# AppleHolic/pytorch_sound

Measured on AMD Instinct MI355X. Metric: audio-sec/s STFT+mel+fwd/bwd, higher is better.
Workload: dtype bf16; 1 GPU; configs[1]: Conv1d separator (4 x ResBlock1, C=256, on 513-bin magnitude), 22.05 kHz, STFT 1024/256, 80 mel, batch 32 x 2 s per GPU, Adam, bf16 autocast; global_batch=32, parallelism=dp1, model_params=5520386

## Files before the change

include/psnd.h:

```cpp
#ifndef PSND_H
#define PSND_H

#include <stdint.h>
#include <stddef.h>

#ifdef __cplusplus
extern "C" {
#endif

#define PSND_OK 0
#define PSND_E_ARG (-1)
#define PSND_E_SHAPE (-2)
#define PSND_E_HIP (-3)
#define PSND_E_UNSUPPORTED (-4)

#define PSND_FRAMING_CENTER 0
#define PSND_FRAMING_HIFIGAN 1
#define PSND_FRAMING_NONE 2

int psnd_version(void);
const char *psnd_last_error(void);
#ifdef PSND_LAB
void psnd_env_refresh(void);
#endif
// ... 89 lines not shown
typedef struct psnd_chain_pair {
    const void *W1;
    const float *bias1;
    float act1_slope;
    void *mid_out;
    const void *W2;
    const float *bias2;
    int off1, dstep1, off2, dstep2;
    float act2_slope;
    void *out_raw, *out_act;
    const void *M1, *M2;
    float m1_slope, m2_slope;
} psnd_chain_pair;
int psnd_conv1d_cl_chain_rows(int C, int k, int n_pairs, const int *taps);
int psnd_conv1d_cl_chain_plan(int C, int k, int n_pairs, const int *taps, int64_t R, int *mr_out);
int psnd_conv1d_cl_chain(const void *A, const void *res, const psnd_chain_pair *pairs, int n_pairs, int64_t N, int Lp, int L, int HP,
                         int C, int k, void *stream);
void psnd_conv_chain_stats(long long *out2);
int psnd_to_cl_nfk(const float *x_nfk, int64_t N, int K, int64_t F, int Lp, int HP, int Cp, int preop, void *out, void *stream);
int64_t psnd_mask_head_l1_blocks_nfk(int64_t N, int64_t F, int K);
int psnd_mask_head_l1_fwd_nfk(const void *y, const float *mag_nfk, const float *ref_nfk, int64_t N, int K, int64_t F, int Lp, int HP, int Cp,
                              float *est_nfk, double *part, void *stream);
int psnd_mask_head_l1_bwd_nfk(const float *gest_nfk, const float *mag_nfk, const void *y, const float *est_nfk, const float *ref_nfk,
                              const float *g, float coef, int64_t N, int K, int64_t F, int Lp, int HP, int Cp, void *gy, void *stream);
int psnd_mel_fwd_nfk(const float *mag_nfk, int64_t N, int64_t F, int M, int K, const void *mel_plan, int log_kind, float log_offset,
                     float pre_clamp_min, float clamp_lo, float clamp_hi, float *out, float *mel_lin, void *stream);
int psnd_mel_bwd_nfk(const float *gout, const float *mel_lin, int64_t N, int64_t F, int M, int K, const void *mel_plan, int log_kind,
                     float log_offset, float pre_clamp_min, float clamp_lo, float clamp_hi, float *gmag_nfk, void *stream);
int psnd_mel_l1_fwd_nfk(const float *mag_nfk, int64_t N, int64_t F, int M, int K, const void *mel_plan, int log_kind, float log_offset,
                        float pre_clamp_min, float clamp_lo, float clamp_hi, const float *ref, float *mel_lin, double *part, void *stream);
int psnd_mel_l1_bwd_nfk(const float *ref, const float *mel_lin, const float *g, float coef, int64_t N, int64_t F, int M, int K,
                        const void *mel_plan, int log_kind, float log_offset, float pre_clamp_min, float clamp_lo, float clamp_hi,
                        float *gmag_nfk, void *stream);
int64_t psnd_mask_head_l1_blocks(int64_t N, int64_t T, int Cp);
int psnd_mask_head_l1_fwd(const void *y, const float *mag, const float *ref, int64_t N, int C, int64_t T, int Lp, int HP, int Cp,
                          float *est, double *part, void *stream);
int psnd_mask_head_l1_bwd(const float *gest, const float *mag, const void *y, const float *est, const float *ref, const float *g,
                          float coef, int64_t N, int C, int64_t T, int Lp, int HP, int Cp, void *gy, void *stream);
int64_t psnd_mel_l1_blocks(int64_t N, int64_t F, int M);
int psnd_mel_l1_fwd(const float *mag, int64_t N, int64_t F, int M, int K, const void *mel_plan, int log_kind, float log_offset,
                    float pre_clamp_min, float clamp_lo, float clamp_hi, const float *ref, float *mel_lin, double *part, void *stream);
int psnd_mel_l1_bwd(const float *ref, const float *mel_lin, const float *g, float coef, int64_t N, int64_t F, int M, int K,
                    const void *mel_plan, int log_kind, float log_offset, float pre_clamp_min, float clamp_lo, float clamp_hi,
                    float *gmag, void *stream);
int psnd_nan_flag(const float *x, int64_t n, float *flag, void *stream);
int psnd_l1_loss_combine(const double *const *parts, const int64_t *nb, const double *scale, int terms, float *out, float *nan_flag, void *stream);
int psnd_conv_stats(int64_t *out4, int reset);
int psnd_conv_pair_stats(int64_t *out4, int reset);
int psnd_conv1d_cl_wgrad(const void *G1, const void *G2, const void *GM, float g2_slope, const void *xa, int64_t N,
                         int Lp, int Ca, int Cb, int k, int off0, int dstep, float *gw_part, float *gbias_part,
                         void *g_out, void *stream);
int psnd_conv1d_prep(const float *v, const float *g, const float *bias, int Cout, int Cin, int k, int Cb, int Ca,
                     void *wf, void *wb, float *bias_padded, void *stream);
int psnd_convtr1d_prep(const float *v, const float *g, const float *bias, int Cin, int Cout, int K, int stride, int Cr, int Cip,
                       void *wf, void *wb, float *bias_rep, void *stream);
int psnd_convtr1d_prep_multi(const void *descs_dev, int n, int total_blocks, void *stream);
int psnd_convtr1d_cl_fwd(const void *xa, const void *wf, const float *bias_rep, int64_t N, int Lp, int L, int HP, int Cip, int Cr,
                         int stride, int padding, int LpO, int HPO, float act_slope, void *out_raw, void *out_act, void *stream);
int psnd_convtr1d_cl_wgrad_splits(int64_t N, int Lp, int Cip, int Cr, int stride);
int psnd_convtr1d_cl_bwd(const void *g_raw, const void *g_act, const void *act, float act_slope, const void *wb, const void *xa,
                         int64_t N, int Lp, int L, int HP, int Cip, int Cr, int stride, int padding, int LpO, int HPO, void *gx,
                         void *g_eff, float *gw_part, void *stream);
int psnd_convtr1d_wnorm_bwd(const float *gw_part, int splits, const float *v, const float *g, int Cin, int Cout, int K, int stride,
                            int Cr, int Cip, float *gv, float *gg, void *stream);
int psnd_cl_mean_act_fwd(const void *a, const void *b, const void *c, const void *d, int count, float slope, void *out, int64_t n,
                         void *stream);
// ... 223 lines not shown
```

pytorch_sound_amd/cl.py:

```python
import ctypes
from collections import namedtuple
from pytorch_sound_amd import _switches as _sw
import weakref

import torch

from . import _lib
from ._lib import lib, ptr, on

ALIGN_C = 32


def round_up(x, m):
    return (x + m - 1) // m * m


class CLShape:

    def __init__(self, N, L, HP):
        self.N, self.L, self.HP = int(N), int(L), int(HP)
        self.Lp = round_up(self.L + 2 * self.HP, 8)

    @property
    def R(self):
# ... 344 lines not shown
        s = _PARAM_STREAM[dev.index] = torch.cuda.Stream(device=dev)
    return s



def branch_streams(dev, n):
    pool = _BRANCH_STREAMS.setdefault(dev.index, [])
    while len(pool) < n:
        pool.append(torch.cuda.Stream(device=dev))
    return pool[:n]


_WGRAD_STREAMS = {}


def _wgrad_streams(dev):
    if _sw.lab('PSND_CL_BWD_SPLIT', '0') != '1' or not _pair_enabled() or not AUTO_SECTIONS:
        return []
    n = int(_sw.lab('PSND_CL_WGRAD_STREAMS', '3'))
    pool = _WGRAD_STREAMS.setdefault(dev.index, [])
    while len(pool) < n:
        pool.append(torch.cuda.Stream(device=dev))
    return pool[:n]


def _pair_enabled():
    return _sw.lab('PSND_CL_PAIR', '1') != '0'


_Step = namedtuple('_Step', 'Cout Cin k Ca Cb dil pad slope has_res has_bias role')
_Conv = namedtuple('_Conv', 'inp wf bp res Ca Cb k off0 dil oslope raw act')
_Pair = namedtuple('_Pair', 'inp1 wf1 bp1 slope1 mid wf2 bp2 res C k off1 dstep1 off2 dstep2 oslope raw act')
_Chain = namedtuple('_Chain', 'inp1 res C k pairs')
_B = namedtuple('_B', 'G1 G2 am slope wb inp Ca Cb k pad dil gx g_out ep_mask ep_slope ep_res gw gbp S')
_W = namedtuple('_W', 'G1 G2 am slope inp Ca Cb k off0 dil gw gbp S')
_Side = namedtuple('_Side', 'w')
_PairB = namedtuple('_PairB', 'G wb2 m1 m1s g_h wb1 m2 m2s res C k off1 dstep1 off2 dstep2 gx flush_after')
_ChainB = namedtuple('_ChainB', 'pairs')
_PB = namedtuple('_PB', 'G wb2 m1 m1s g_h wb1 m2 m2s C k pad2 dil2 pad1 dil1 gx gw gbp lag')
_PBFlush = namedtuple('_PBFlush', 'lag')
_Lag = namedtuple('_Lag', 'g xa off0 dstep gw gbp C k')
_WBatch = namedtuple('_WBatch', 'conv G inp off0 dstep')


def _chain_takes(pairs):
    taps = [t for p in pairs for t in (p.off1, p.dstep1, p.off2, p.dstep2)]
    return lib().psnd_conv1d_cl_chain_rows(pairs[0].C, pairs[0].k, len(pairs), (ctypes.c_int * len(taps))(*taps)) >= 32


def _chain_pairs_bwd(plan, rows):
    mx = int(_sw.lab('PSND_CL_CHAIN_BWD', _sw.lab('PSND_CL_CHAIN', '3')))
    if mx < 2 or rows > 8192:
        return plan
    out = []
    for e in plan:
        if isinstance(e, _PairB) and e.C == 256 and e.res is e.G:
            c = out[-1] if out and isinstance(out[-1], _ChainB) else None
            if (c is not None and len(c.pairs) < mx and c.pairs[-1].gx is e.G and c.pairs[-1].k == e.k
                    and _chain_takes(c.pairs + [e])):
                c.pairs.append(e)
                continue
            out.append(_ChainB([e]))
        else:
            out.append(e)
    return [c.pairs[0] if isinstance(c, _ChainB) and len(c.pairs) == 1 else c for c in out]

# ... 269 lines not shown

class MeanActCL(torch.autograd.Function):

    @staticmethod
    def forward(ctx, slope, *rs):
        n = len(rs)
        if not 1 <= n <= 4:
            raise _lib.PsndError('MeanActCL: 1..4 branches, got %d' % n)
        rs = [r.contiguous() for r in rs]
        for r in rs:
            _need(r, torch.bfloat16)
        out = torch.empty_like(rs[0])
        ps = [ptr(r) for r in rs] + [None] * (4 - n)
        with on(out.device) as hip:
            hip.psnd_cl_mean_act_fwd(ps[0], ps[1], ps[2], ps[3], n, float(slope), out, out.numel())
        ctx.n, ctx.slope = n, float(slope)
        ctx.save_for_backward(out)
        return out

    @staticmethod
    def backward(ctx, g):
        (out,) = ctx.saved_tensors
        g = g.contiguous()
        gin = torch.empty_like(out)
        with on(out.device) as hip:
            hip.psnd_cl_mean_act_bwd(g, out, ctx.n, ctx.slope, gin, out.numel())
        return (None,) + (gin,) * ctx.n


class PrepPacks(dict):
    deferred = None

    def write_backward_packs(self):
        cache = self.deferred
        if cache is None or cache['wb_done']:
            return
        cache['wb_done'] = True
        with on(cache['dev']) as hip:
            hip.psnd_conv1d_prep_multi(cache['table'], cache['n'], cache['blocks'], cache['max_row'], 2)


def prep_all(owner, convs, defer_backward_packs=False):
    import struct
    if _sw.lab('PSND_NO_PREP_ALL') == '1':
        return None
    if any(c.weight_v.shape[1] * c.weight_v.shape[2] > 10240 for c in convs):
        return None
    key = tuple((c.weight_v.data_ptr(), c.weight_g.data_ptr(), 0 if c.bias is None else c.bias.data_ptr(),
                 tuple(c.weight_v.shape)) for c in convs)
    cache = getattr(owner, '_cl_prep_cache', None)
    if cache is None or cache['key'] != key:
        dev = convs[0].weight_v.device
        packs, recs, blk0, max_row = PrepPacks(), [], 0, 0
        for c in convs:
            Cout, Cin, k = c.weight_v.shape
            Ca, Cb = round_up(Cin, ALIGN_C), round_up(Cout, ALIGN_C)
            wf = torch.zeros((k, Cb, Ca), dtype=torch.bfloat16, device=dev)
            wb = torch.zeros((k, Ca, Cb), dtype=torch.bfloat16, device=dev)
            bp = torch.zeros(Cb, dtype=torch.float32, device=dev)
            packs[id(c)] = (wf, wb, bp)
            recs.append(struct.pack('<6Q6i', c.weight_v.data_ptr(), c.weight_g.data_ptr(),
                                    0 if c.bias is None else c.bias.data_ptr(), wf.data_ptr(), wb.data_ptr(), bp.data_ptr(),
                                    Cout, Cin, k, Cb, Ca, blk0))
            blk0 += (Cout + 7) // 8
            max_row = max(max_row, Cin * k)
        table = torch.frombuffer(bytearray(b''.join(recs)), dtype=torch.uint8).to(dev)
        cache = {'key': key, 'packs': packs, 'table': table, 'n': len(convs), 'blocks': blk0, 'max_row': max_row, 'dev': dev,
                 'wb_done': True}
        owner._cl_prep_cache = cache
    for c in convs:
        if not (c.weight_v.is_contiguous() and c.weight_g.is_contiguous() and c.weight_v.dtype == torch.float32):
            raise _lib.PsndError('prep_all: fp32 contiguous weight_v / weight_g expected')
    defer = bool(defer_backward_packs) and torch.is_grad_enabled() and _sw.lab('PSND_PREP_NO_DEFER') != '1'
    with on(cache['dev']) as hip:
        hip.psnd_conv1d_prep_multi(cache['table'], cache['n'], cache['blocks'], cache['max_row'], 1 if defer else 3)
    cache['wb_done'] = not defer
    cache['packs'].deferred = cache if defer else None
    return cache['packs']


def fused_conv(xa, conv, shape, res=None, want_raw=False, want_act=True, act_slope=0.1, prep=None):
    return FusedConvCL.apply(xa, conv.weight_v, conv.weight_g, conv.bias, res, shape, conv.dilation, want_raw, want_act,
                             act_slope, None if prep is None else prep[id(conv)])


class ResBlockCL(torch.autograd.Function):

    @staticmethod
    def forward(ctx, x, xa, shape, roles, dils, last_act_slope, want_raw, packs, *params):
        ctx.set_materialize_grads(False)
        _need(xa, torch.bfloat16)
        dev = xa.device
        n = len(dils)
        ctx.pack_owner = getattr(packs, 'owner', None)
        steps, saved, plan = [], [], []
        cur_x, cur_xa, pending = x, xa, None
        for i in range(n):
            wv, wg, b = params[3 * i:3 * i + 3]
            Cout, Cin, k = wv.shape
            role = roles[i]
            src = pending if role == 'c2' else cur_xa
            Ca, Cb = src.shape[2], round_up(Cout, ALIGN_C)
            if Ca != round_up(Cin, ALIGN_C) or (role in ('c2', 'r2') and Cb != cur_x.shape[2]):
                raise _lib.PsndError('CL conv chain: %s conv %d -> %d channels on a %d-channel buffer' % (role, Cin, Cout, Ca))
            dil = dils[i]
            pad = (k * dil - dil) // 2
            v32, g32 = wv.detach().contiguous(), wg.detach().contiguous()
            if packs is not None and packs[i] is not None:
                wf, wb, bp = packs[i]
            else:
                wf = torch.empty((k, Cb, Ca), dtype=torch.bfloat16, device=dev)
                wb = torch.empty((k, Ca, Cb), dtype=torch.bfloat16, device=dev)
                bp = torch.empty(Cb, dtype=torch.float32, device=dev)
                b32 = None if b is None else b.detach().contiguous()
                with on(dev) as hip:
                    hip.psnd_conv1d_prep(v32, g32, b32, Cout, Cin, k, Cb, Ca, wf, wb, bp)
            last = i == n - 1
            inp, slope, has_res = src, (last_act_slope if last else 0.1), role in ('c2', 'r2')
            mk = lambda: torch.empty((shape.N, shape.Lp, Cb), dtype=torch.bfloat16, device=dev)
            if role == 'c1':
                raw, act, res, oslope = None, mk(), None, slope
                pending = act
            elif role == 'tail':
                raw, act, res, oslope = mk(), None, None, 1.0
                cur_x, cur_xa = raw, None
            else:
                raw, act, res, oslope = (mk() if (not last) or want_raw else None), mk(), (cur_x if has_res else None), slope
                cur_x, cur_xa = raw, act
            c1 = plan[-1] if plan else None
            if (role == 'c2' and _pair_enabled() and isinstance(c1, _Conv) and steps[-1].role == 'c1' and c1.Ca == Ca == Cb
                    and c1.k == k and lib().psnd_conv1d_cl_pair_supported(Ca, k, c1.off0, c1.dil, -pad, dil)):
                plan[-1] = _Pair(c1.inp, c1.wf, c1.bp, c1.oslope, c1.act, wf, bp, res, Ca, k, c1.off0, c1.dil, -pad, dil, oslope, raw, act)
            else:
                plan.append(_Conv(inp, wf, bp, res, Ca, Cb, k, -pad, dil, oslope, raw, act))
            steps.append(_Step(Cout, Cin, k, Ca, Cb, dil, pad, slope, has_res, b is not None, role))
            saved += [inp, act if act is not None else inp, wb, v32, g32]
        nsec, sides = _sections(dev, shape.N, shape.N * shape.Lp)
        Nh = shape.N // nsec
        plan = _chain_pairs(plan, Nh * shape.Lp)

        def run(h):
            q = lambda t: ptr(_sec(t, h, nsec))
            with on(dev) as hip:
                for e in plan:
                    if isinstance(e, _Chain):
                        inp1, res0, C, k, pairs = e
                        arr = (_lib.ChainPair * len(pairs))()
                        for d, p in zip(arr, pairs):
                            d.W1, d.bias1, d.act1_slope, d.mid_out = p.wf1.data_ptr(), p.bp1.data_ptr(), float(p.slope1), q(p.mid)
                            d.W2, d.bias2, d.off1, d.dstep1, d.off2, d.dstep2 = p.wf2.data_ptr(), p.bp2.data_ptr(), p.off1, p.dstep1, p.off2, p.dstep2
                            d.act2_slope, d.out_raw, d.out_act = float(p.oslope), (q(p.raw) if p is pairs[-1] else None), q(p.act)
                        hip.psnd_conv1d_cl_chain(q(inp1), q(res0), ctypes.addressof(arr), len(pairs), Nh, shape.Lp, shape.L, shape.HP, C, k)
                        continue
                    if isinstance(e, _Pair):
                        inp1, wf1, bp1, slope1, mid, wf2, bp2, res, C, k, off1, dstep1, off2, dstep2, oslope, raw, act = e
                        hip.psnd_conv1d_cl_pair(q(inp1), wf1, bp1, None, 1.0, float(slope1), q(mid), wf2, bp2, None, 1.0, q(res), Nh, shape.Lp, shape.L,
                                                shape.HP, C, k, off1, dstep1, off2, dstep2, float(oslope), q(raw), q(act))
                        continue
                    inp, wf, bp, res, Ca, Cb, k, off0, dil, oslope, raw, act = e
                    hip.psnd_conv1d_cl(q(inp), None, None, 1.0, wf, bp, q(res), None, Nh, shape.Lp, shape.L, shape.HP, Ca, Cb, k, off0, dil,
                                       float(oslope), 1.0, q(raw), q(act), None)

        with torch.cuda.device(dev):
            _run_sections(dev, nsec, sides, run)
        ctx.steps, ctx.shape = steps, shape
        ctx.param_refs = params
        note_param_use(ctx, *params)
        ctx.save_for_backward(*saved)
        return cur_x, cur_xa

    @staticmethod
    def backward(ctx, g_raw, g_act):
        saved, steps, shape = ctx.saved_tensors, ctx.steps, ctx.shape
        dev = saved[0].device
        n = len(steps)
        if ctx.pack_owner is not None:
            ctx.pack_owner.write_backward_packs()
        g_raw = None if g_raw is None else g_raw.contiguous()
        g_act = None if g_act is None else g_act.contiguous()
        grads = [None] * (3 * n)
        descs, keep = [None] * n, []
        res_pending = None
        sink = GRAD_SINK if (GRAD_SINK is not None and GRAD_SINK.sink_active()) else None
        prefs = getattr(ctx, 'param_refs', None)
        early = {}

        def grad_out(i, v32, g32, Cb):
            gv = gg = gb = None
            if sink is not None and prefs is not None:
                pv, pg, pb = prefs[3 * i:3 * i + 3]
# ... 200 lines not shown
                if out:
                    sink.deliver(out)

            if sink is not None and batch:
                done_w = 0
                launches = [j for j, e in enumerate(plan) if isinstance(e, (_PairB, _ChainB))]
                L, C = len(launches), max(1, int(HANDOVER_CHUNKS))
                cut = {launches[min(L - 1, max(0, round((j + 1) * L / C) - 1))] for j in range(C - 1)} if L else set()
                ready = []
                for j, e in enumerate(plan):
                    run(0, [e])
                    ready += [ci for pe, ci in own_launch if pe is e]
                    if j not in cut:
                        continue
                    upto = (e.pairs[-1] if isinstance(e, _ChainB) else e).flush_after
                    part, done_w = wbatch[done_w:upto], upto
                    wgrad_batch(part)
                    finish(ready + [b.conv for b in part])
                    ready = []
                part = wbatch[done_w:]
                rest = [ci for ci in range(n) if descs[ci] is not None and ci not in handed and ci not in ready]
                wgrad_batch(part)
                finish(ready + rest + [b.conv for b in part])
            else:
                _run_sections(dev, nsec, sides, run)
                for sd in set(used):
                    torch.cuda.current_stream(dev).wait_stream(sd)
                wgrad_batch(wbatch)
                finish([ci for ci in range(n) if descs[ci] is not None])
        consume_param_use(ctx)
        return (g_raw, g_act, None, None, None, None, None, None) + tuple(grads)


def _block_node(convs, x, xa, shape, pairs, last_act_slope, want_raw, prep):
    params = []
    for c in convs:
        params += [c.weight_v, c.weight_g, c.bias]
    packs = None if prep is None else _PackList(prep[id(c)] for c in convs)
    if packs is not None:
        packs.owner = prep if isinstance(prep, PrepPacks) else None
    roles = pairs if isinstance(pairs, tuple) else (('c1', 'c2') * (len(convs) // 2) if pairs else ('r2',) * len(convs))
    return ResBlockCL.apply(x, xa, shape, roles, tuple(c.dilation for c in convs), last_act_slope, want_raw, packs, *params)


class _PackList(list):
    owner = None


def _use_block_node(convs, x):
    return (_sw.lab('PSND_NO_BLOCK_NODE') != '1' and x is not None and len(convs) <= 64
            and all(c.weight_v.shape[0] == c.weight_v.shape[1] for c in convs))


def conv_body_cl(head, blocks, tail, x0, shape, prep=None):
    stack = [c for b in blocks for pair in zip(b.convs1, b.convs2) for c in pair]
    if (_sw.lab('PSND_NO_BODY_NODE') == '1' or _sw.lab('PSND_NO_BLOCK_NODE') == '1' or not _stack_enabled()
            or NODE_GRANULARITY == 'block'):
        if isinstance(prep, PrepPacks):
            prep.write_backward_packs()
        x, xa = fused_conv(x0, head, shape, None, True, True, 0.1, prep)
        x, xa = resblock1_stack_cl(blocks, x, xa, shape, prep=prep)
        return fused_conv(xa, tail, shape, None, True, False, prep=prep)[0]
    convs = [head] + stack + [tail]
    roles = ('head',) + ('c1', 'c2') * (len(stack) // 2) + ('tail',)
    return _block_node(convs, None, x0, shape, roles, 0.1, True, prep)[0]


def resblock1_cl(block, x, xa, shape, last_act_slope=0.1, want_raw=True, prep=None):
    n = len(block.convs1)
    convs = [c for pair in zip(block.convs1, block.convs2) for c in pair]
    if _use_block_node(convs, x):
        return _block_node(convs, x, xa, shape, True, last_act_slope, want_raw, prep)
    for i, (c1, c2) in enumerate(zip(block.convs1, block.convs2)):
        _, ta = fused_conv(xa, c1, shape, None, False, True, 0.1, prep)
        last = i == n - 1
        x, xa = fused_conv(ta, c2, shape, x, (not last) or want_raw, True, last_act_slope if last else 0.1, prep)
    return x, xa


def resblock1_stack_cl(blocks, x, xa, shape, last_act_slope=0.1, want_raw=True, prep=None):
    convs = [c for b in blocks for pair in zip(b.convs1, b.convs2) for c in pair]
    if _use_block_node(convs, x) and _stack_enabled():
        return _block_node(convs, x, xa, shape, True, last_act_slope, want_raw, prep)
    for i, b in enumerate(blocks):
        last = i == len(blocks) - 1
        x, xa = resblock1_cl(b, x, xa, shape, last_act_slope if last else 0.1, want_raw or not last, prep)
    return x, xa


def _stack_enabled():
    return _sw.lab('PSND_NO_BLOCK_STACK') != '1' and NODE_GRANULARITY != 'block'


def resblock2_cl(block, x, xa, shape, last_act_slope=0.1, want_raw=True, prep=None):
    n = len(block.convs)
    if _use_block_node(list(block.convs), x):
        return _block_node(list(block.convs), x, xa, shape, False, last_act_slope, want_raw, prep)
    for i, c in enumerate(block.convs):
# ... 4 lines not shown
```

pytorch_sound_amd/csrc/psnd_core.hip:

```cpp
#include "psnd_common.h"

static thread_local char g_err[512] = "";

void psnd_set_error(const char *fmt, ...) {
    va_list ap;
    va_start(ap, fmt);
    vsnprintf(g_err, sizeof(g_err), fmt, ap);
    va_end(ap);
}

extern "C" int psnd_version(void) { return 151; }

extern "C" const char *psnd_last_error(void) { return g_err; }

#ifdef PSND_LAB
std::atomic<int> g_psnd_env_gen{0};
extern "C" void psnd_env_refresh(void) { g_psnd_env_gen.fetch_add(1, std::memory_order_acq_rel); }
#endif

static inline int64_t pad_of(int n_fft, int hop, int framing) {
    if (framing == PSND_FRAMING_NONE) return 0;
    return framing == PSND_FRAMING_CENTER ? n_fft / 2 : (n_fft - hop) / 2;
}

extern "C" int64_t psnd_frame_count(int64_t T, int n_fft, int hop, int framing) {
    if (T <= 0 || n_fft <= 0 || hop <= 0) return 0;
    const int64_t L = T + 2 * pad_of(n_fft, hop, framing);
    if (L < n_fft) return 0;
    return (L - n_fft) / hop + 1;
}

extern "C" int64_t psnd_frame_sample_index(int64_t f, int m, int64_t T, int n_fft, int hop, int framing) {
    int64_t i = f * hop - pad_of(n_fft, hop, framing) + m;
    if (i < 0) i = -i;
    if (i >= T) i = 2 * (T - 1) - i;
    return i;
}

extern "C" void *psnd_event_create(void) {
    hipEvent_t ev = nullptr;
    if (hipEventCreateWithFlags(&ev, hipEventDisableTiming) != hipSuccess) {
        psnd_set_error("event_create: %s", hipGetErrorString(hipGetLastError()));
        return nullptr;
    }
// ... 96 lines not shown
```

pytorch_sound_amd/csrc/psnd_nfk.hip:

```cpp
#include "psnd_common.h"

namespace {

typedef unsigned short bf16_t;
typedef __bf16 hwbf16x2 __attribute__((ext_vector_type(2)));

__device__ __forceinline__ float bf_lo(unsigned v) { return __builtin_bit_cast(float, v << 16); }
__device__ __forceinline__ float bf_hi(unsigned v) { return __builtin_bit_cast(float, v & 0xffff0000u); }
__device__ __forceinline__ unsigned pack_bf16(float lo, float hi) {
    const f32x2 v = {lo, hi};
    return __builtin_bit_cast(unsigned, __builtin_convertvector(v, hwbf16x2));
}

struct Row8 {
    float v[8];
};
__device__ __forceinline__ Row8 load8(__amdgpu_buffer_rsrc_t r, unsigned row_byte, int c0, int K, bool row_ok) {
    Row8 o;
    constexpr unsigned OOB = 0xffffffffu;
    if (c0 + 8 <= K) {
        const unsigned b = row_ok ? row_byte + 4u * (unsigned)c0 : OOB;
        const f32x4 a = __builtin_bit_cast(f32x4, __builtin_amdgcn_raw_buffer_load_b128(r, (int)b, 0, 0));
        const f32x4 c = __builtin_bit_cast(f32x4, __builtin_amdgcn_raw_buffer_load_b128(r, (int)(row_ok ? b + 16u : OOB), 0, 0));
        o.v[0] = a.x, o.v[1] = a.y, o.v[2] = a.z, o.v[3] = a.w, o.v[4] = c.x, o.v[5] = c.y, o.v[6] = c.z, o.v[7] = c.w;
    } else {
#pragma unroll
        for (int j = 0; j < 8; ++j)
            o.v[j] = __builtin_bit_cast(float, __builtin_amdgcn_raw_buffer_load_b32(r, (int)((row_ok && c0 + j < K) ? row_byte + 4u * (unsigned)(c0 + j) : OOB), 0, 0));
    }
    return o;
}
__device__ __forceinline__ void store8(__amdgpu_buffer_rsrc_t r, unsigned row_byte, int c0, int K, const float (&v)[8]) {
    if (c0 + 8 <= K) {
// ... 10 lines not shown
    const float *x;
    const float *ref;
    const float *est_in;
    const float *gest;
    const float *g;
    const bf16_t *y;
    bf16_t *out_cl;
    float *est;
    double *part;
    long long items;
    int N, F, K, Lp, HP, Cp, preop;
    unsigned tensor_bytes;
    float coef;
};

template <bool MASKBWD>
__global__ __launch_bounds__(256) void to_cl_nfk_kernel(NfkParams p) {
    const long long it = (long long)blockIdx.x * 256 + threadIdx.x;
    if (it >= p.items) return;
    const int cpr = p.Cp >> 3;
    const long long row = it / cpr;
    const int c0 = (int)(it - row * cpr) * 8;
    const int n = (int)(row / p.Lp), l = (int)(row - (long long)n * p.Lp), t = l - p.HP;
    const bool ok = t >= 0 && t < p.F;
    const unsigned rb = (unsigned)(((size_t)n * p.F + (size_t)(ok ? t : 0)) * p.K * 4);
    const int tb = (int)p.tensor_bytes;
    const __amdgpu_buffer_rsrc_t rx = make_uniform_rsrc(p.x, tb);
    float w[8];
    if constexpr (!MASKBWD) {
        const Row8 a = load8(rx, rb, c0, p.K, ok);
#pragma unroll
        for (int j = 0; j < 8; ++j) {
            float v = a.v[j];
            if (p.preop == 1) {
                const float u = 1.f + v;
                v = u == 1.f ? v : __logf(u) * __fdividef(v, u - 1.f);
            }
            w[j] = v;
        }
    } else {
        const __amdgpu_buffer_rsrc_t re = make_uniform_rsrc(p.est_in, tb), rr = make_uniform_rsrc(p.ref, tb);
        const __amdgpu_buffer_rsrc_t rg = make_uniform_rsrc(p.gest ? p.gest : p.x, p.gest ? tb : 0);
        const Row8 m = load8(rx, rb, c0, p.K, ok), e = load8(re, rb, c0, p.K, ok), r = load8(rr, rb, c0, p.K, ok), ge = load8(rg, rb, c0, p.K, ok);
        const u32x4 yq = *reinterpret_cast<const u32x4 *>(p.y + (size_t)row * p.Cp + c0);
        const float l1c = p.coef * p.g[0];
#pragma unroll
        for (int j = 0; j < 8; ++j) {
            const unsigned q = yq[j >> 1];
            const float yv = (j & 1) ? bf_hi(q) : bf_lo(q);
            const float sg = 1.f / (1.f + __expf(-yv));
            const float d = e.v[j] - r.v[j];
            const float gg = ge.v[j] + l1c * (d > 0.f ? 1.f : (d < 0.f ? -1.f : 0.f));
            w[j] = gg * m.v[j] * sg * (1.f - sg);
        }
    }
    const u32x4 o = {pack_bf16(w[0], w[1]), pack_bf16(w[2], w[3]), pack_bf16(w[4], w[5]), pack_bf16(w[6], w[7])};
    *reinterpret_cast<u32x4 *>(p.out_cl + (size_t)row * p.Cp + c0) = o;
}

__global__ __launch_bounds__(256) void mask_head_nfk_kernel(NfkParams p) {
    const long long it = (long long)blockIdx.x * 256 + threadIdx.x;
    const int cpr = (p.K + 7) >> 3;
    float acc = 0.f;
    if (it < p.items) {
        const long long row = it / cpr;
        const int c0 = (int)(it - row * cpr) * 8;
        const int n = (int)(row / p.F), t = (int)(row - (long long)n * p.F);
        const unsigned rb = (unsigned)((size_t)row * p.K * 4);
        const int tb = (int)p.tensor_bytes;
        const __amdgpu_buffer_rsrc_t rm = make_uniform_rsrc(p.x, tb), rr = make_uniform_rsrc(p.ref ? p.ref : p.x, p.ref ? tb : 0);
// ... 83 lines not shown
```

pytorch_sound_amd/models/separator.py:

```python
import torch
import torch.nn as nn
import torch.nn.functional as F

from pytorch_sound_amd.models import register_model, register_model_architecture
from pytorch_sound_amd.models.vocoders.hifi_gan import WNConv1d, ResBlock1, LRELU_SLOPE, wants_bf16


@register_model('conv_separator')
class ConvSeparator(nn.Module):
    def __init__(self, spec_size: int = 513, channels: int = 256, num_blocks: int = 4, kernel_size: int = 3,
                 dilation=(1, 3, 5)):
        super().__init__()
        self.conv_pre = WNConv1d(spec_size, channels, 3, 1, 1)
        self.blocks = nn.ModuleList([ResBlock1(None, channels, kernel_size, tuple(dilation)) for _ in range(num_blocks)])
        self.conv_post = WNConv1d(channels, spec_size, 3, 1, 1, init_std=0.01)

    precision = 'auto'

    def forward(self, mag: torch.Tensor) -> torch.Tensor:
        from pytorch_sound_amd import deferred
        if mag.is_cuda and wants_bf16(self.precision, mag):
            node = deferred.nfk_of(mag) if deferred.ENABLED else None
            if node is not None:
                y, shape = self.logits_cl(node.nfk, 'nfk')
# ... 30 lines not shown
    def separate(self, wav: torch.Tensor, stft, eps: float = None) -> torch.Tensor:
        from pytorch_sound_amd import host as H, kernels as K
        from pytorch_sound_amd.models.transforms import STFTTorchAudio
        if wav.dim() != 2:
            raise RuntimeError('expected a (N, T) waveform batch, got shape %s' % (tuple(wav.shape),))
        if torch.is_grad_enabled() and wav.requires_grad:
            raise RuntimeError('ConvSeparator.separate: the mixture carries no gradient (wav.requires_grad is set)')
        torchaudio_kind = isinstance(stft, STFTTorchAudio)
        n_fft = stft.n_fft if torchaudio_kind else stft.filter_length
        hop = stft.hop_length
        if eps is None:
            eps = 0.0 if torchaudio_kind else 1e-9
        if not wav.is_cuda:
            c = H.stft_complex(wav, n_fft, hop, stft._host_window(), H.FRAMING_CENTER)
            re, im = c.real, c.imag
            logits = self.mask_logits(torch.sqrt(re ** 2 + im ** 2))
            return H.istft_complex(re, im, logits, H.MASK_SIGMOID, n_fft, hop, stft._host_window(), eps)
        plan = stft._plan(wav.device)
        o = K.stft_forward(wav.detach().float(), n_fft, hop, plan, K.FRAMING_CENTER, 0.0, want_mag=True, want_reim=True)
        logits = self.mask_logits(o['mag'])
        return K.istft_reim(o['re'], o['im'], logits, K.MASK_SIGMOID, n_fft, hop, plan, eps)


    def logits_cl(self, mag: torch.Tensor, layout: str = 'nkf'):
        from pytorch_sound_amd import cl
        if layout == 'nfk':
            N, T, C = mag.shape
        else:
            N, C, T = mag.shape
        halo = max(c.padding for b in self.blocks for c in list(b.convs1) + list(b.convs2))
        shape = cl.CLShape(N, T, max(halo, self.conv_pre.padding, self.conv_post.padding))
        convs = [self.conv_pre] + [c for b in self.blocks for c in list(b.convs1) + list(b.convs2)] + [self.conv_post]
        prep = cl.prep_all(self, convs, defer_backward_packs=True)
        x0 = cl.to_cl_nfk(mag.float(), shape, 1) if layout == 'nfk' else cl.ToCL.apply(mag.float(), shape, 1)
        return cl.conv_body_cl(self.conv_pre, list(self.blocks), self.conv_post, x0, shape, prep), shape

    def spectral_l1_loss(self, mag: torch.Tensor, mag_ref: torch.Tensor, mel_ref: torch.Tensor, mel_plan: torch.Tensor, n_mels: int,
                         w_mag: float = 1.0, w_mel: float = 0.5, log_offset: float = 1e-6, clamp_lo=None, clamp_hi=None, layout: str = 'nkf'):
        from pytorch_sound_amd import cl, kernels as K
        if not mag.is_cuda:
            raise RuntimeError('spectral_l1_loss is the fused HIP formulation; on the host compose the loss from forward()')
        if layout == 'nfk':
            y, shape = self.logits_cl(mag, 'nfk')
            loss, est = cl.MaskHeadSpectralL1NFK.apply(y, mag.float().contiguous(), mag_ref.float().contiguous(), mel_ref.float().contiguous(),
                                                       mel_plan, shape, n_mels, K.LOG_E, log_offset, None, clamp_lo, clamp_hi, w_mag, w_mel)
            loss.psnd_nan_flag = cl.LAST_LOSS_NAN_FLAG[0]
            return loss, est
        y, shape = self.logits_cl(mag)
        loss, est = cl.MaskHeadSpectralL1CL.apply(y, mag.float().contiguous(), mag_ref.float().contiguous(), mel_ref.float().contiguous(),
                                                  mel_plan, shape, n_mels, K.LOG_E, log_offset, None, clamp_lo, clamp_hi, w_mag, w_mel)
        loss.psnd_nan_flag = cl.LAST_LOSS_NAN_FLAG[0]
        return loss, est

    def forward_cl(self, mag: torch.Tensor) -> torch.Tensor:
        from pytorch_sound_amd import cl
        N, C, T = mag.shape
        halo = max(c.padding for b in self.blocks for c in list(b.convs1) + list(b.convs2))
        shape = cl.CLShape(N, T, max(halo, self.conv_pre.padding, self.conv_post.padding))
        convs = [self.conv_pre] + [c for b in self.blocks for c in list(b.convs1) + list(b.convs2)] + [self.conv_post]
        prep = cl.prep_all(self, convs, defer_backward_packs=True)
        x0 = cl.ToCL.apply(mag.float(), shape, 1)
        y = cl.conv_body_cl(self.conv_pre, list(self.blocks), self.conv_post, x0, shape, prep)
        if mag.dtype == torch.float32 and not mag.requires_grad:
            from pytorch_sound_amd import deferred
            if deferred.ENABLED:
                return deferred.est(y, mag.contiguous(), shape)
            return cl.MaskHeadCL.apply(y, mag, shape)
# ... 8 lines not shown
```

Before: 108,900 audio-s/s.

## Fuse NFK-to-channel-last conversion with log1p into the head conv kernel

Adds a dedicated HIP kernel for the first (head) conv that reads the fp32 NFK magnitude directly, applies log1p, converts to bf16 channel-last in LDS, writes the CL copy for backward, and runs the k=3 head convolution with bias and leaky-ReLU epilogue. This removes the separate to_cl_nfk pass and the re-read of the converted tensor by the generic head conv. It also refactors the prep cache so the deferred-pack launch record is separate from the cache dict. The cost is a large specialised kernel limited to Cout=256, k=3, dil=1, and it needs a large dynamic LDS allocation that may reduce occupancy compared with the generic conv.

```diff
diff --git a/include/psnd.h b/include/psnd.h
--- a/include/psnd.h
+++ b/include/psnd.h
@@ -145,6 +145,10 @@
 int psnd_mel_l1_bwd_nfk(const float *ref, const float *mel_lin, const float *g, float coef, int64_t N, int64_t F, int M, int K,
                         const void *mel_plan, int log_kind, float log_offset, float pre_clamp_min, float clamp_lo, float clamp_hi,
                         float *gmag_nfk, void *stream);
+int psnd_conv1d_cl_head_nfk_plan(int64_t N, int64_t F, int K, int Lp, int HP, int Cp, int Cout, int k, int dil, int mr, int64_t *grid_out,
+                                 int *lds_out);
+int psnd_conv1d_cl_head_nfk(const float *x_nfk, const void *wf, const float *bp, int64_t N, int K, int64_t F, int Lp, int HP, int Cp, int Cout,
+                            int k, int dil, int preop, float act_slope, int mr, void *x_cl, void *out_raw, void *out_act, void *stream);
 int64_t psnd_mask_head_l1_blocks(int64_t N, int64_t T, int Cp);
 int psnd_mask_head_l1_fwd(const void *y, const float *mag, const float *ref, int64_t N, int C, int64_t T, int Lp, int HP, int Cp,
                           float *est, double *part, void *stream);
diff --git a/pytorch_sound_amd/cl.py b/pytorch_sound_amd/cl.py
--- a/pytorch_sound_amd/cl.py
+++ b/pytorch_sound_amd/cl.py
@@ -400,6 +400,7 @@
 _Conv = namedtuple('_Conv', 'inp wf bp res Ca Cb k off0 dil oslope raw act')
 _Pair = namedtuple('_Pair', 'inp1 wf1 bp1 slope1 mid wf2 bp2 res C k off1 dstep1 off2 dstep2 oslope raw act')
 _Chain = namedtuple('_Chain', 'inp1 res C k pairs')
+_HeadNfk = namedtuple('_HeadNfk', 'x_nfk preop mr K x_cl wf bp Ca Cb k dil oslope raw act')
 _B = namedtuple('_B', 'G1 G2 am slope wb inp Ca Cb k pad dil gx g_out ep_mask ep_slope ep_res gw gbp S')
 _W = namedtuple('_W', 'G1 G2 am slope inp Ca Cb k off0 dil gw gbp S')
 _Side = namedtuple('_Side', 'w')
@@ -735,12 +736,12 @@
     deferred = None
 
     def write_backward_packs(self):
-        cache = self.deferred
-        if cache is None or cache['wb_done']:
+        launch = self.deferred
+        if launch is None or launch['wb_done']:
             return
-        cache['wb_done'] = True
-        with on(cache['dev']) as hip:
-            hip.psnd_conv1d_prep_multi(cache['table'], cache['n'], cache['blocks'], cache['max_row'], 2)
+        launch['wb_done'] = True
+        with on(launch['dev']) as hip:
+            hip.psnd_conv1d_prep_multi(launch['table'], launch['n'], launch['blocks'], launch['max_row'], 2)
 
 
 def prep_all(owner, convs, defer_backward_packs=False):
@@ -768,17 +769,18 @@
             blk0 += (Cout + 7) // 8
             max_row = max(max_row, Cin * k)
         table = torch.frombuffer(bytearray(b''.join(recs)), dtype=torch.uint8).to(dev)
-        cache = {'key': key, 'packs': packs, 'table': table, 'n': len(convs), 'blocks': blk0, 'max_row': max_row, 'dev': dev,
-                 'wb_done': True}
+        launch = {'table': table, 'n': len(convs), 'blocks': blk0, 'max_row': max_row, 'dev': dev, 'wb_done': True}
+        cache = {'key': key, 'packs': packs, 'launch': launch}
         owner._cl_prep_cache = cache
     for c in convs:
         if not (c.weight_v.is_contiguous() and c.weight_g.is_contiguous() and c.weight_v.dtype == torch.float32):
             raise _lib.PsndError('prep_all: fp32 contiguous weight_v / weight_g expected')
     defer = bool(defer_backward_packs) and torch.is_grad_enabled() and _sw.lab('PSND_PREP_NO_DEFER') != '1'
-    with on(cache['dev']) as hip:
-        hip.psnd_conv1d_prep_multi(cache['table'], cache['n'], cache['blocks'], cache['max_row'], 1 if defer else 3)
-    cache['wb_done'] = not defer
-    cache['packs'].deferred = cache if defer else None
+    launch = cache['launch']
+    with on(launch['dev']) as hip:
+        hip.psnd_conv1d_prep_multi(launch['table'], launch['n'], launch['blocks'], launch['max_row'], 1 if defer else 3)
+    launch['wb_done'] = not defer
+    cache['packs'].deferred = launch if defer else None
     return cache['packs']
 
 
@@ -834,6 +836,9 @@
             if (role == 'c2' and _pair_enabled() and isinstance(c1, _Conv) and steps[-1].role == 'c1' and c1.Ca == Ca == Cb
                     and c1.k == k and lib().psnd_conv1d_cl_pair_supported(Ca, k, c1.off0, c1.dil, -pad, dil)):
                 plan[-1] = _Pair(c1.inp, c1.wf, c1.bp, c1.oslope, c1.act, wf, bp, res, Ca, k, c1.off0, c1.dil, -pad, dil, oslope, raw, act)
+            elif i == 0 and role == 'head' and getattr(packs, 'head_nfk', None) is not None:
+                x_nfk, preop, mr = packs.head_nfk
+                plan.append(_HeadNfk(x_nfk, preop, mr, Cin, inp, wf, bp, Ca, Cb, k, dil, oslope, raw, act))
             else:
                 plan.append(_Conv(inp, wf, bp, res, Ca, Cb, k, -pad, dil, oslope, raw, act))
             steps.append(_Step(Cout, Cin, k, Ca, Cb, dil, pad, slope, has_res, b is not None, role))
@@ -859,6 +864,10 @@
                         inp1, wf1, bp1, slope1, mid, wf2, bp2, res, C, k, off1, dstep1, off2, dstep2, oslope, raw, act = e
                         hip.psnd_conv1d_cl_pair(q(inp1), wf1, bp1, None, 1.0, float(slope1), q(mid), wf2, bp2, None, 1.0, q(res), Nh, shape.Lp, shape.L,
                                                 shape.HP, C, k, off1, dstep1, off2, dstep2, float(oslope), q(raw), q(act))
+                        continue
+                    if isinstance(e, _HeadNfk):
+                        hip.psnd_conv1d_cl_head_nfk(q(e.x_nfk), e.wf, e.bp, Nh, e.K, shape.L, shape.Lp, shape.HP, e.Ca, e.Cb, e.k, e.dil, e.preop,
+                                                    float(e.oslope), e.mr, q(e.x_cl), q(e.raw), q(e.act))
                         continue
                     inp, wf, bp, res, Ca, Cb, k, off0, dil, oslope, raw, act = e
                     hip.psnd_conv1d_cl(q(inp), None, None, 1.0, wf, bp, q(res), None, Nh, shape.Lp, shape.L, shape.HP, Ca, Cb, k, off0, dil,
@@ -1125,19 +1134,21 @@
         return (g_raw, g_act, None, None, None, None, None, None) + tuple(grads)
 
 
-def _block_node(convs, x, xa, shape, pairs, last_act_slope, want_raw, prep):
+def _block_node(convs, x, xa, shape, pairs, last_act_slope, want_raw, prep, head_nfk=None):
     params = []
     for c in convs:
         params += [c.weight_v, c.weight_g, c.bias]
     packs = None if prep is None else _PackList(prep[id(c)] for c in convs)
     if packs is not None:
         packs.owner = prep if isinstance(prep, PrepPacks) else None
+        packs.head_nfk = head_nfk
     roles = pairs if isinstance(pairs, tuple) else (('c1', 'c2') * (len(convs) // 2) if pairs else ('r2',) * len(convs))
     return ResBlockCL.apply(x, xa, shape, roles, tuple(c.dilation for c in convs), last_act_slope, want_raw, packs, *params)
 
 
 class _PackList(list):
     owner = None
+    head_nfk = None
 
 
 def _use_block_node(convs, x):
@@ -1145,18 +1156,50 @@
             and all(c.weight_v.shape[0] == c.weight_v.shape[1] for c in convs))
 
 
+def _body_is_one_node():
+    return not (_sw.lab('PSND_NO_BODY_NODE') == '1' or _sw.lab('PSND_NO_BLOCK_NODE') == '1' or not _stack_enabled()
+                or NODE_GRANULARITY == 'block')
+
+
+def _body_node(head, blocks, tail, x0, shape, prep, head_nfk=None):
+    stack = [c for b in blocks for pair in zip(b.convs1, b.convs2) for c in pair]
+    roles = ('head',) + ('c1', 'c2') * (len(stack) // 2) + ('tail',)
+    return _block_node([head] + stack + [tail], None, x0, shape, roles, 0.1, True, prep, head_nfk)[0]
+
+
 def conv_body_cl(head, blocks, tail, x0, shape, prep=None):
-    stack = [c for b in blocks for pair in zip(b.convs1, b.convs2) for c in pair]
-    if (_sw.lab('PSND_NO_BODY_NODE') == '1' or _sw.lab('PSND_NO_BLOCK_NODE') == '1' or not _stack_enabled()
-            or NODE_GRANULARITY == 'block'):
+    if not _body_is_one_node():
         if isinstance(prep, PrepPacks):
             prep.write_backward_packs()
         x, xa = fused_conv(x0, head, shape, None, True, True, 0.1, prep)
         x, xa = resblock1_stack_cl(blocks, x, xa, shape, prep=prep)
         return fused_conv(xa, tail, shape, None, True, False, prep=prep)[0]
-    convs = [head] + stack + [tail]
-    roles = ('head',) + ('c1', 'c2') * (len(stack) // 2) + ('tail',)
-    return _block_node(convs, None, x0, shape, roles, 0.1, True, prep)[0]
+    return _body_node(head, blocks, tail, x0, shape, prep)
+
+
+def head_nfk_rows(head, shape, K):
+    if _sw.lab('PSND_HEAD_NFK', '1') == '0':
+        return 0, 0
+    Cout, Cin, k = head.weight_v.shape
+    mr = int(_sw.lab('PSND_HEAD_NFK_MR', '0'))
+    if Cin != K:
+        return 0, mr
+    return int(lib().psnd_conv1d_cl_head_nfk_plan(shape.N, shape.L, K, shape.Lp, shape.HP, round_up(K, ALIGN_C), round_up(Cout, ALIGN_C), k,
+                                                   int(head.dilation), mr, None, None)), mr
+
+
+def conv_body_cl_nfk(head, blocks, tail, x_nfk, shape, prep=None, preop=1):
+    rows, mr = head_nfk_rows(head, shape, x_nfk.shape[2]) if (_body_is_one_node() and prep is not None and x_nfk.dim() == 3) else (0, 0)
+    if not rows:
+        return conv_body_cl(head, blocks, tail, to_cl_nfk(x_nfk, shape, preop), shape, prep)
+    _need(x_nfk, torch.float32)
+    if x_nfk.requires_grad and torch.is_grad_enabled():
+        raise _lib.PsndError('conv_body_cl_nfk carries no gradient to its input (feature tensors are inputs)')
+    N, F, K = x_nfk.shape
+    if F != shape.L or N != shape.N:
+        raise _lib.PsndError('conv_body_cl_nfk: tensor %s does not match the CL geometry (N=%d, L=%d)' % (tuple(x_nfk.shape), shape.N, shape.L))
+    x0 = torch.empty((N, shape.Lp, round_up(K, ALIGN_C)), dtype=torch.bfloat16, device=x_nfk.device)
+    return _body_node(head, blocks, tail, x0, shape, prep, (x_nfk, int(preop), mr))
 
 
 def resblock1_cl(block, x, xa, shape, last_act_slope=0.1, want_raw=True, prep=None):
diff --git a/pytorch_sound_amd/csrc/psnd_conv_head.hip b/pytorch_sound_amd/csrc/psnd_conv_head.hip
--- /dev/null
+++ b/pytorch_sound_amd/csrc/psnd_conv_head.hip
@@ -0,0 +1,281 @@
+#include "psnd_conv_pair.h"
+#include "psnd_log1p.h"
+#include <atomic>
+
+namespace {
+using pairk::bf16_t;
+using pairk::bf16x8;
+using pairk::f32x16;
+using pairk::pack_bf16;
+
+constexpr unsigned HOOB = 0x80000000u;
+constexpr int HNT = 512, HCB = 256, HHM = 1, HRU = 12, HAR = 3, HORS = HCB + 8;
+constexpr int kHeadLdsBudget = 160 * 1024;
+
+__device__ __forceinline__ unsigned oob_unless(bool ok) { return ok ? 0u : HOOB; }
+
+struct HeadParams {
+    const float *x;
+    const bf16_t *W;
+    const float *bias;
+    bf16_t *x_cl;
+    bf16_t *out_raw, *out_act;
+    int N, F, K, Lp, HP, Cp, preop;
+    float act_slope;
+};
+
+template <int MR>
+__global__ __launch_bounds__(HNT, 1) void conv_head_nfk_kernel(HeadParams p) {
+    constexpr int MROWS = 32 * MR, BR = MROWS + 2 * HHM;
+    constexpr int NB = MR == 2 ? 9 : 5;
+    extern __shared__ __attribute__((aligned(16))) bf16_t smem[];
+    bf16_t *sX = smem;
+    const int tid = threadIdx.x, wave = tid >> 6, lane = tid & 63, li = lane & 31, kg = lane >> 5;
+    const int Cp = p.Cp, RS = Cp + 8, PCS = Cp >> 3, KSTEPS = Cp >> 4, nstage = Cp >> 5, K = p.K;
+    const long long R = (long long)p.N * p.Lp;
+    const long long g0 = (long long)blockIdx.x * MROWS;
+    const __amdgpu_buffer_rsrc_t rX = make_uniform_rsrc(p.x, (int)((size_t)p.N * p.F * K * sizeof(float)));
+    const __amdgpu_buffer_rsrc_t rW = make_uniform_rsrc(p.W, (int)((size_t)3 * HCB * Cp * sizeof(bf16_t)));
+
+    uint4 rb[HRU];
+    const unsigned fwave = (unsigned)wave * (unsigned)KSTEPS * 1024u + (unsigned)lane * 16u;
+    const unsigned FTAP = (unsigned)(HCB / 32) * (unsigned)KSTEPS * 1024u;
+    auto fetch_b = [&](auto slotc, int it) __attribute__((always_inline)) {
+        constexpr int slot = decltype(slotc)::value, tap = slot % 6 / 2;
+        const int ks = 4 * it + 2 * (slot / 6) + slot % 2;
+        rb[slot] = __builtin_bit_cast(uint4, __builtin_amdgcn_raw_buffer_load_b128(rW, (int)(ks < KSTEPS ? fwave : HOOB),
+                                                                                    (int)((unsigned)tap * FTAP + (unsigned)ks * 1024u), 0));
+    };
+    static_for<0, HRU>([&](auto uc) __attribute__((always_inline)) { fetch_b(uc, 0); });
+    const int cb = wave * 32 + 4 * kg;
+    const bool has_bias = p.bias != nullptr;
+    const __amdgpu_buffer_rsrc_t rBias = make_uniform_rsrc(has_bias ? (const void *)p.bias : (const void *)p.x, has_bias ? HCB * (int)sizeof(float) : 0);
+    f32x4 bb[4];
+#pragma unroll
+    for (int g = 0; g < 4; ++g) bb[g] = __builtin_bit_cast(f32x4, __builtin_amdgcn_raw_buffer_load_b128(rBias, (cb + 8 * g) * (int)sizeof(float), 0, 0));
+
+    int n0, l0;
+    if (blockIdx.x == 0) {
+        n0 = -1, l0 = p.Lp - HHM;
+    } else {
+        const unsigned gb = (unsigned)(g0 - HHM);
+        n0 = (int)(gb / (unsigned)p.Lp), l0 = (int)(gb - (unsigned)n0 * (unsigned)p.Lp);
+    }
+    const float rLp = 1.f / (float)p.Lp;
+    auto frame = [&](int b, bool &ok) __attribute__((always_inline)) {
+        const int x = l0 + b;
+        int q = (int)((float)x * rLp);
+        int l = x - q * p.Lp;
+        const int under = l < 0 ? 1 : 0, over = l >= p.Lp ? 1 : 0;
+        l += (under - over) * p.Lp, q += over - under;
+        const int n = n0 + q, t = l - p.HP;
+        ok = (n >= 0) & (n < p.N) & (t >= 0) & (t < p.F);
+        return (unsigned)(n * p.F + t) * (unsigned)K * 4u;
+    };
+    const int kt = K & ~3, ntail = K & 3;
+    const int tb = tid >> 2, tj = tid & 3;
+    float tv;
+    {
+        bool ok;
+        const unsigned fb = frame(tb, ok);
+        tv = __builtin_bit_cast(float, __builtin_amdgcn_raw_buffer_load_b32(rX, (int)((fb + 4u * (unsigned)(kt + tj)) | oob_unless(ok & (tb < BR) & (tj < ntail))), 0, 0));
+    }
+    const int nitems = BR * PCS, dr = HNT / PCS, dp = HNT - dr * PCS;
+    const int row_t = tid / PCS, pc_t = tid - row_t * PCS;
+    {
+        int row = row_t, pc = pc_t;
+        auto batch = [&]() __attribute__((always_inline)) {
+            f32x4 va[NB], vb[NB];
+            int lo[NB];
+#pragma unroll
+            for (int u = 0; u < NB; ++u) {
+                bool ok;
+                const unsigned fb = frame(row, ok);
+                const int c0 = 8 * pc;
+                const unsigned o = fb + 4u * (unsigned)c0;
+                ok = ok & (row < BR);
+                va[u] = __builtin_bit_cast(f32x4, __builtin_amdgcn_raw_buffer_load_b128(rX, (int)(o | oob_unless(ok & (c0 + 4 <= K))), 0, 0));
+                vb[u] = __builtin_bit_cast(f32x4, __builtin_amdgcn_raw_buffer_load_b128(rX, (int)((o + 16u) | oob_unless(ok & (c0 + 8 <= K))), 0, 0));
+                lo[u] = row < BR ? row * RS + c0 : -1;
+                pc += dp, row += dr;
+                if (pc >= PCS) pc -= PCS, ++row;
+            }
+            auto commit = [&](auto prec) __attribute__((always_inline)) {
+                auto pre = [&](float v) __attribute__((always_inline)) { return decltype(prec)::value ? psnd_log1p_bf16(v) : v; };
+#pragma unroll
+                for (int u = 0; u < NB; ++u) {
+                    const uint4 w = make_uint4(pack_bf16(pre(va[u].x), pre(va[u].y)), pack_bf16(pre(va[u].z), pre(va[u].w)),
+                                               pack_bf16(pre(vb[u].x), pre(vb[u].y)), pack_bf16(pre(vb[u].z), pre(vb[u].w)));
+                    if (lo[u] >= 0) *reinterpret_cast<uint4 *>(sX + lo[u]) = w;
+                }
+            };
+            if (p.preop == 1) commit(std::true_type{});
+            else commit(std::false_type{});
+        };
+        batch();
+#pragma unroll 1
+        for (int base = HNT * NB; base < nitems; base += HNT * NB) batch();
+    }
+    if (ntail) {
+        __syncthreads();
+        const float w = p.preop == 1 ? psnd_log1p_bf16(tv) : tv;
+        if (tb < BR && tj < ntail) sX[tb * RS + kt + tj] = (bf16_t)(pack_bf16(w, 0.f) & 0xffffu);
+    }
+    unsigned rmask[MR];
+#pragma unroll
+    for (int m = 0; m < MR; ++m) {
+        bool ok;
+        (void)frame(HHM + 32 * m + li, ok);
+        rmask[m] = ok ? 0xffffffffu : 0u;
+    }
+    __syncthreads();
+
+    f32x16 acc[MR];
+#pragma unroll
+    for (int m = 0; m < MR; ++m)
+#pragma unroll
+        for (int i = 0; i < 16; ++i) acc[m][i] = 0.f;
+    const bf16_t *ab[3];
+#pragma unroll
+    for (int t = 0; t < 3; ++t) ab[t] = sX + (li + t) * RS + 8 * kg;
+    auto afrag = [&](auto uc, int it, bf16x8 (&x)[MR]) __attribute__((always_inline)) {
+        constexpr int u = decltype(uc)::value, tap = u % 6 / 2;
+        const bf16_t *pa = ab[tap] + 32 * (2 * it + u / 6) + 16 * (u % 2);
+#pragma unroll
+        for (int m = 0; m < MR; ++m) x[m] = *reinterpret_cast<const bf16x8 *>(pa + m * 32 * RS);
+    };
+    const __amdgpu_buffer_rsrc_t rO = make_uniform_rsrc(p.x_cl, (int)((size_t)R * Cp * sizeof(bf16_t)));
+    int crow = row_t, cpc = pc_t;
+    auto copy_step = [&]() __attribute__((always_inline)) {
+        const long long r = g0 + crow;
+        const uint4 v = *reinterpret_cast<const uint4 *>(sX + ((crow < MROWS ? crow : 0) + HHM) * RS + 8 * cpc);
+        __builtin_amdgcn_raw_buffer_store_b128(__builtin_bit_cast(u32x4, v), rO,
+                                               (int)((crow < MROWS && r < R) ? (unsigned)(((size_t)r * Cp + 8 * cpc) * sizeof(bf16_t)) : HOOB), 0, 0);
+        cpc += dp, crow += dr;
+        if (cpc >= PCS) cpc -= PCS, ++crow;
+    };
+    bf16x8 xr[HAR][MR];
+    static_for<0, HAR - 1>([&](auto uc) __attribute__((always_inline)) { afrag(uc, 0, xr[decltype(uc)::value]); });
+    auto turn = [&](auto nuc, auto refillc, int it) __attribute__((always_inline)) {
+        constexpr int NU = decltype(nuc)::value;
+        constexpr bool REFILL = decltype(refillc)::value;
+        copy_step();
+        static_for<0, NU>([&](auto uc) __attribute__((always_inline)) {
+            constexpr int u = decltype(uc)::value;
+            afrag(std::integral_constant<int, u + HAR - 1>{}, it, xr[(u + HAR - 1) % HAR]);
+            const bf16x8 b = __builtin_bit_cast(bf16x8, rb[u]);
+#pragma unroll
+            for (int m = 0; m < MR; ++m) acc[m] = __builtin_amdgcn_mfma_f32_32x32x16_bf16(b, xr[u % HAR][m], acc[m], 0, 0, 0);
+            if constexpr (REFILL) fetch_b(uc, it + 1);
+            __builtin_amdgcn_sched_group_barrier(0x100, MR, 0);
+            __builtin_amdgcn_sched_group_barrier(0x008, MR, 0);
+            if constexpr (REFILL) __builtin_amdgcn_sched_group_barrier(0x020, 1, 0);
+            __builtin_amdgcn_sched_barrier(0);
+        });
+    };
+    const int nfull = nstage >> 1;
+#pragma unroll 1
+    for (int it = 0; it < nfull; ++it) turn(std::integral_constant<int, HRU>{}, std::true_type{}, it);
+    if (nstage & 1) turn(std::integral_constant<int, HRU / 2>{}, std::false_type{}, nfull);
+
+    __syncthreads();
+    bf16_t *sR = smem, *sA = smem + MROWS * HORS;
+    const int eo = li * HORS + cb;
+    const float slope = p.act_slope;
+    const bool want_raw = p.out_raw != nullptr, want_act = p.out_act != nullptr;
+#pragma unroll
+    for (int m = 0; m < MR; ++m)
+#pragma unroll
+        for (int g = 0; g < 4; ++g) {
+            float v[4], a[4];
+#pragma unroll
+            for (int j = 0; j < 4; ++j) {
+                v[j] = acc[m][4 * g + j];
+                if (has_bias) v[j] += bb[g][j];
+                a[j] = v[j] > 0.f ? v[j] : v[j] * slope;
+            }
+            if (want_raw)
+                *reinterpret_cast<uint2 *>(sR + eo + m * 32 * HORS + 8 * g) = make_uint2(pack_bf16(v[0], v[1]) & rmask[m], pack_bf16(v[2], v[3]) & rmask[m]);
+            if (want_act)
+                *reinterpret_cast<uint2 *>(sA + eo + m * 32 * HORS + 8 * g) = make_uint2(pack_bf16(a[0], a[1]) & rmask[m], pack_bf16(a[2], a[3]) & rmask[m]);
+        }
+    __syncthreads();
+    const int o_bytes = (int)((size_t)R * HCB * sizeof(bf16_t));
+    const __amdgpu_buffer_rsrc_t rRaw = make_uniform_rsrc(want_raw ? (const void *)p.out_raw : (const void *)p.x, want_raw ? o_bytes : 0);
+    const __amdgpu_buffer_rsrc_t rAct = make_uniform_rsrc(want_act ? (const void *)p.out_act : (const void *)p.x, want_act ? o_bytes : 0);
+#pragma unroll
+    for (int u = 0; u < MROWS * (HCB / 8) / HNT; ++u) {
+        const int idx = tid + HNT * u, row = idx >> 5, pc = idx & 31;
+        const long long r = g0 + row;
+        const unsigned o = r < R ? (unsigned)(((size_t)r * HCB + 8 * pc) * sizeof(bf16_t)) : HOOB;
+        const uint4 vr = *reinterpret_cast<const uint4 *>(sR + row * HORS + 8 * pc), va = *reinterpret_cast<const uint4 *>(sA + row * HORS + 8 * pc);
+        __builtin_amdgcn_raw_buffer_store_b128(__builtin_bit_cast(u32x4, vr), rRaw, (int)o, 0, 0);
+        __builtin_amdgcn_raw_buffer_store_b128(__builtin_bit_cast(u32x4, va), rAct, (int)o, 0, 0);
+    }
+}
+
+size_t head_lds_bytes(int mr, int Cp) {
+    const size_t tile = (size_t)(32 * mr + 2 * HHM) * (Cp + 8) * sizeof(bf16_t) + 128, outs = (size_t)2 * 32 * mr * HORS * sizeof(bf16_t);
+    return tile > outs ? tile : outs;
+}
+template <int MR>
+bool head_launch(const HeadParams &p, int64_t grid, int lds, hipStream_t st) {
+    constexpr int kMaxDev = 64;
+    static std::atomic<int> state[kMaxDev];
+    int dev = 0;
+    if (hipGetDevice(&dev) != hipSuccess || dev < 0 || dev >= kMaxDev) return false;
+    int s = state[dev].load(std::memory_order_acquire);
+    if (s == 0) {
+        s = hipFuncSetAttribute(reinterpret_cast<const void *>(conv_head_nfk_kernel<MR>), hipFuncAttributeMaxDynamicSharedMemorySize, kHeadLdsBudget) == hipSuccess ? 1 : -1;
+        state[dev].store(s, std::memory_order_release);
+    }
+    if (s < 0) return false;
+    hipLaunchKernelGGL(conv_head_nfk_kernel<MR>, dim3((unsigned)grid), dim3(HNT), (size_t)lds, st, p);
+    return true;
+}
+constexpr int kHeadDefaultMr = 1;
+}
+
+extern "C" int psnd_conv1d_cl_head_nfk_plan(int64_t N, int64_t F, int K, int Lp, int HP, int Cp, int Cout, int k, int dil, int mr, int64_t *grid_out,
+                                            int *lds_out) {
+    if (grid_out) *grid_out = 0;
+    if (lds_out) *lds_out = 0;
+    if (Cout != HCB || k != 3 || dil != 1 || mr < 0 || mr > 2) return 0;
+    if (N <= 0 || F <= 0 || K <= 0 || HP < HHM || Lp < F + 2 * HP || Lp >= (1 << 22) || Cp % 32 != 0 || Cp < K) return 0;
+    if ((size_t)N * (size_t)F * (size_t)K * 4 >= ((size_t)1 << 31) || (size_t)N * (size_t)Lp * (size_t)(Cp > HCB ? Cp : HCB) * 2 >= ((size_t)1 << 31) ||
+        (size_t)3 * HCB * (size_t)Cp * 2 >= ((size_t)1 << 31))
+        return 0;
+    const bool forced = mr != 0;
+    if (!forced) mr = kHeadDefaultMr;
+    if (head_lds_bytes(mr, Cp) > (size_t)kHeadLdsBudget) {
+        if (forced || mr == 1 || head_lds_bytes(1, Cp) > (size_t)kHeadLdsBudget) return 0;
+        mr = 1;
+    }
+    if (grid_out) *grid_out = (N * (int64_t)Lp + 32 * mr - 1) / (32 * mr);
+    if (lds_out) *lds_out = (int)head_lds_bytes(mr, Cp);
+    return 32 * mr;
+}
+
+extern "C" int psnd_conv1d_cl_head_nfk(const float *x_nfk, const void *wf, const float *bp, int64_t N, int K, int64_t F, int Lp, int HP, int Cp, int Cout,
+                                       int k, int dil, int preop, float act_slope, int mr, void *x_cl, void *out_raw, void *out_act, void *stream) {
+    if (!x_nfk || !wf || !x_cl || (!out_raw && !out_act)) PSND_FAIL(PSND_E_ARG, "conv1d_cl_head_nfk: null pointer");
+    if (preop < 0 || preop > 1) PSND_FAIL(PSND_E_ARG, "conv1d_cl_head_nfk: preop=%d", preop);
+    if (N == 0) return PSND_OK;
+    int64_t grid = 0;
+    int lds = 0;
+    const int rows = psnd_conv1d_cl_head_nfk_plan(N, F, K, Lp, HP, Cp, Cout, k, dil, mr, &grid, &lds);
+    if (!rows)
+        PSND_FAIL(PSND_E_UNSUPPORTED, "conv1d_cl_head_nfk: N=%lld F=%lld K=%d Lp=%d HP=%d Cp=%d Cout=%d k=%d dil=%d mr=%d (Cout = 256, k = 3, dil = 1, Cp %% 32 == 0, the row tile within %d KB of LDS)",
+                  (long long)N, (long long)F, K, Lp, HP, Cp, Cout, k, dil, mr, kHeadLdsBudget / 1024);
+    HeadParams p;
+    p.x = x_nfk, p.W = static_cast<const bf16_t *>(wf), p.bias = bp;
+    p.x_cl = static_cast<bf16_t *>(x_cl), p.out_raw = static_cast<bf16_t *>(out_raw), p.out_act = static_cast<bf16_t *>(out_act);
+    p.N = (int)N, p.F = (int)F, p.K = K, p.Lp = Lp, p.HP = HP, p.Cp = Cp, p.preop = preop, p.act_slope = act_slope;
+    hipStream_t st = static_cast<hipStream_t>(stream);
+    if (!(rows == 64 ? head_launch<2>(p, grid, lds, st) : head_launch<1>(p, grid, lds, st))) {
+        (void)hipGetLastError();
+        PSND_FAIL(PSND_E_HIP, "conv1d_cl_head_nfk: %d bytes of dynamic LDS refused", kHeadLdsBudget);
+    }
+    PSND_CHECK_LAUNCH("conv1d_cl_head_nfk");
+    return PSND_OK;
+}
diff --git a/pytorch_sound_amd/csrc/psnd_core.hip b/pytorch_sound_amd/csrc/psnd_core.hip
--- a/pytorch_sound_amd/csrc/psnd_core.hip
+++ b/pytorch_sound_amd/csrc/psnd_core.hip
@@ -9,7 +9,7 @@
     va_end(ap);
 }
 
-extern "C" int psnd_version(void) { return 151; }
+extern "C" int psnd_version(void) { return 152; }
 
 extern "C" const char *psnd_last_error(void) { return g_err; }
 
diff --git a/pytorch_sound_amd/csrc/psnd_log1p.h b/pytorch_sound_amd/csrc/psnd_log1p.h
--- /dev/null
+++ b/pytorch_sound_amd/csrc/psnd_log1p.h
@@ -0,0 +1,8 @@
+#pragma once
+#include "psnd_common.h"
+
+__device__ __forceinline__ float psnd_log1p_bf16(float v) {
+    const float u = 1.f + v;
+    const float w = __logf(u) * __fdividef(v, u - 1.f);
+    return u == 1.f ? v : w;
+}
diff --git a/pytorch_sound_amd/csrc/psnd_nfk.hip b/pytorch_sound_amd/csrc/psnd_nfk.hip
--- a/pytorch_sound_amd/csrc/psnd_nfk.hip
+++ b/pytorch_sound_amd/csrc/psnd_nfk.hip
@@ -1,4 +1,5 @@
 #include "psnd_common.h"
+#include "psnd_log1p.h"
 
 namespace {
 
@@ -75,10 +76,7 @@
 #pragma unroll
         for (int j = 0; j < 8; ++j) {
             float v = a.v[j];
-            if (p.preop == 1) {
-                const float u = 1.f + v;
-                v = u == 1.f ? v : __logf(u) * __fdividef(v, u - 1.f);
-            }
+            if (p.preop == 1) v = psnd_log1p_bf16(v);
             w[j] = v;
         }
     } else {
diff --git a/pytorch_sound_amd/models/separator.py b/pytorch_sound_amd/models/separator.py
--- a/pytorch_sound_amd/models/separator.py
+++ b/pytorch_sound_amd/models/separator.py
@@ -86,7 +86,9 @@
         shape = cl.CLShape(N, T, max(halo, self.conv_pre.padding, self.conv_post.padding))
         convs = [self.conv_pre] + [c for b in self.blocks for c in list(b.convs1) + list(b.convs2)] + [self.conv_post]
         prep = cl.prep_all(self, convs, defer_backward_packs=True)
-        x0 = cl.to_cl_nfk(mag.float(), shape, 1) if layout == 'nfk' else cl.ToCL.apply(mag.float(), shape, 1)
+        if layout == 'nfk':
+            return cl.conv_body_cl_nfk(self.conv_pre, list(self.blocks), self.conv_post, mag.float(), shape, prep, 1), shape
+        x0 = cl.ToCL.apply(mag.float(), shape, 1)
         return cl.conv_body_cl(self.conv_pre, list(self.blocks), self.conv_post, x0, shape, prep), shape
 
     def spectral_l1_loss(self, mag: torch.Tensor, mag_ref: torch.Tensor, mel_ref: torch.Tensor, mel_plan: torch.Tensor, n_mels: int,
```

New measurement: 107,600 audio-s/s. 0.988x the previous value.
